# SonSang/dmesh_renderer

Hardware: AMD Instinct MI355X
Metric: fwd+bwd Mpixels/sec @1080p, 500k tris; grad max-abs-err vs ref (higher is better)
Workload: dtype f32

## Files before the change

dmesh_renderer_amd/csrc/dmr_api.hip:

```cpp
#include <algorithm>
#include <atomic>
#include <chrono>
#include <cstdio>
#include <cstdlib>
#include <cstring>
#include <functional>
#include <map>
#include <mutex>
#include <string>
#include <vector>

#include "dmr_kernels.hpp"

namespace {

thread_local std::string g_err;

int fail(const std::string& m) { g_err = m; return 1; }

#define DMR_HIP(expr)                                                                           \
    do {                                                                                        \
        hipError_t e_ = (expr);                                                                 \
        if (e_ != hipSuccess) return fail(std::string(#expr) + ": " + hipGetErrorString(e_));   \
    } while (0)

constexpr size_t ALIGN = 256;
inline size_t up(size_t n) { return (n + ALIGN - 1) & ~(ALIGN - 1); }

struct Carver {
    char* base; size_t off;
    explicit Carver(void* b) : base(reinterpret_cast<char*>(b)), off(0) {}
    template <class T> T* take(size_t count) {
        T* p = base ? reinterpret_cast<T*>(base + off) : nullptr;
        off += up(count * sizeof(T));
        return p;
    }
};

struct PointState { float4* vproj; };
struct FaceState { uint2* rect; float* key_depth; float* max_depth; uint32_t* tiles_touched; void* facerec; void* colrec; void* tetrec; };
struct ImageState {
    uint32_t* tile_count; uint32_t* tile_offset; uint32_t* tile_cursor; int* num_rendered;
    float* final_T; float* final_prev_T; uint32_t* n_contrib;
    uint32_t* tile_hits; uint32_t* tile_bound; uint32_t* scan_tmp; uint32_t* hit_offset; uint32_t* tile_used; unsigned long long* hit_total; uint32_t* tile_order;
    int32_t* first_face; int32_t* first_tet; int32_t* last_face; int32_t* last_tet; uint8_t* is_active;
    float* mats;
    int* seed;
    unsigned long long* mask_offset;
    dmr::TetSeq* seq;
};
struct BinningState {
    uint64_t* keys; uint32_t* face_list; uint32_t capacity; unsigned long long mask_offset, mask_first;
    char* base; unsigned long long seq_offset; uint32_t seq_steps;
};

size_t carve_point(void* b, size_t BP, PointState& s) { Carver c(b); s.vproj = c.take<float4>(BP); return c.off; }
size_t carve_face(void* b, size_t BF, size_t F, size_t T, bool tet, FaceState& s) {
    Carver c(b);
    s.rect = c.take<uint2>(BF); s.key_depth = c.take<float>(BF);
    s.max_depth = tet ? c.take<float>(BF) : nullptr;
    s.tiles_touched = c.take<uint32_t>(BF);
    s.facerec = s.colrec = s.tetrec = nullptr;
    if (tet) {
        s.facerec = c.take<char>(F * dmr::tet_facerec_bytes());
        s.colrec = c.take<char>(F * dmr::tet_colrec_bytes());
        s.tetrec = c.take<char>(T * dmr::tet_tetrec_bytes());
    }
    return c.off;
}
size_t carve_image(void* b, size_t B, size_t ntiles, size_t npix, bool tet, ImageState& s) {
    Carver c(b);
    s.mats = c.take<float>(64 * B);
    s.seed = c.take<int>(1);
    s.mask_offset = c.take<unsigned long long>(2);
    s.tile_count = c.take<uint32_t>(ntiles); s.tile_hits = c.take<uint32_t>(ntiles); s.tile_bound = c.take<uint32_t>(ntiles);
    s.scan_tmp = c.take<uint32_t>(dmr::scan_tmp_words((int)ntiles));
    s.hit_offset = c.take<uint32_t>(ntiles + 1); s.tile_used = c.take<uint32_t>(ntiles); s.hit_total = c.take<unsigned long long>(1);
    s.tile_offset = c.take<uint32_t>(ntiles + 1);
    s.tile_cursor = c.take<uint32_t>(ntiles); s.num_rendered = c.take<int>(1);
    s.tile_order = c.take<uint32_t>(ntiles);
    s.final_T = c.take<float>(npix); s.final_prev_T = c.take<float>(npix); s.n_contrib = c.take<uint32_t>(npix);
    if (tet) {
        s.first_face = c.take<int32_t>(npix); s.first_tet = c.take<int32_t>(npix);
        s.last_face = c.take<int32_t>(npix); s.last_tet = c.take<int32_t>(npix);
        s.is_active = c.take<uint8_t>(npix);
        s.seq = c.take<dmr::TetSeq>(1);
    } else {
        s.first_face = s.first_tet = s.last_face = s.last_tet = nullptr; s.is_active = nullptr;
        s.seq = nullptr;
    }
    return c.off;
}
size_t carve_binning(void* b, size_t R, size_t mask_tiles, size_t seq_tiles, size_t seq_steps, BinningState& s) {
    Carver c(b);
    s.face_list = c.take<uint32_t>(R); s.keys = c.take<uint64_t>(R);
    s.capacity = (uint32_t)std::min<size_t>(R, 0xffffffffu);
    s.mask_offset = c.off;
    s.mask_first = dmr::mask_first_slots(R, mask_tiles);
    if (mask_tiles && R > 0) c.take<uint4>(dmr::mask_slots(R, mask_tiles) * 256);
    s.base = reinterpret_cast<char*>(b); s.seq_offset = c.off; s.seq_steps = (uint32_t)seq_steps;
    if (seq_steps) c.take<char>(dmr::tet_seq_bytes(seq_tiles, seq_steps));
    return c.off;
}

struct Dims { int gx, gy, r0, r1, ntiles; size_t BP, BF, npix; };

dmr_scene canonical(const dmr_scene* s, const float* mats) {
    dmr_scene c = *s;
    const size_t n = 16 * (size_t)s->B;
    c.mv_mats = mats; c.proj_mats = mats + n; c.inv_mv_mats = mats + 2 * n; c.inv_proj_mats = mats + 3 * n;
    c.mats_transposed = 0;
    return c;
}

int check_scene(const dmr_scene* s, bool tet, Dims& d) {
    if (!s) return fail("null scene");
    if (s->B <= 0 || s->W <= 0 || s->H <= 0 || s->P < 0 || s->F < 0 || s->T < 0) return fail("bad dimensions");
    if ((int64_t)s->B * s->P > INT32_MAX || (int64_t)s->B * s->F > INT32_MAX || (int64_t)s->B * s->W * s->H > INT32_MAX)
        return fail("problem too large for 32-bit indexing");
    d.gx = (s->W + dmr::TILE - 1) / dmr::TILE;
    d.gy = (s->H + dmr::TILE - 1) / dmr::TILE;
    if (d.gx > 65535 || d.gy > 65535) return fail("image too large (tile coordinates must fit 16 bits)");
    d.r0 = s->row_begin; d.r1 = s->row_end;
    if (d.r0 == 0 && d.r1 == 0) d.r1 = d.gy;
    d.r0 = std::max(0, std::min(d.gy, d.r0));
    d.r1 = std::max(d.r0, std::min(d.gy, d.r1));
    d.ntiles = s->B * d.gx * d.gy;
    d.BP = (size_t)s->B * s->P; d.BF = (size_t)s->B * s->F; d.npix = (size_t)s->B * s->W * s->H;
    if (tet && s->F > 0 && s->P > 0 && (!s->tets || !s->face_tets || !s->tet_faces)) return fail("tet topology missing");
    if (tet && s->F >= (1 << 28)) return fail("too many faces for the tet renderer (face ids must fit 28 bits)");
    return 0;
}
// ... 38 lines not shown
    auto it = g_overflow.find(dev);
    if (it != g_overflow.end()) return it->second;
    if (!create) return nullptr;
    void* p = nullptr;
    if (hipHostMalloc(&p, 64, hipHostMallocCoherent | hipHostMallocPortable) != hipSuccess) return nullptr;
    *reinterpret_cast<volatile uint32_t*>(p) = 0u;
    return g_overflow[dev] = reinterpret_cast<uint32_t*>(p);
}

bool stream_is_capturing(hipStream_t st) {
    hipStreamCaptureStatus cs = hipStreamCaptureStatusNone;
    if (hipStreamIsCapturing(st, &cs) != hipSuccess) { (void)hipGetLastError(); return false; }
    return cs != hipStreamCaptureStatusNone;
}

struct SizeKey {
    int v[7];
    bool operator<(const SizeKey& o) const { return memcmp(v, o.v, sizeof(v)) < 0; }
};
struct SizeGuess { double rendered_per_face = 0.0, hits_per_face = 0.0; uint32_t* seq_steps = nullptr; };
std::mutex g_size_mu;
std::map<SizeKey, SizeGuess> g_size_cache;
std::atomic<uint64_t> g_redo_count{0};
int size_bucket(size_t BF) { int b = 0; while ((BF >> (b + 1)) != 0) b++; return b; }
SizeKey size_key(const dmr_scene* s, bool tet, const Dims& d) {
    return SizeKey{{s->B, s->W, s->H, d.r0, d.r1, tet ? 1 : 0, size_bucket(d.BF)}};
}
double lookup_estimate(const SizeKey& key, double SizeGuess::* field) {
    for (int db : {0, -1, 1}) {
        SizeKey k = key; k.v[6] += db;
        auto it = g_size_cache.find(k);
        if (it != g_size_cache.end() && it->second.*field > 0.0) return it->second.*field;
    }
    return 0.0;
}
uint64_t padded(uint64_t n) { return n + n / 4 + 4096; }

int run_forward(const dmr_scene* s, bool tet, const Dims& d, dmr_alloc_fn alloc, void* ctx, hipStream_t st,
                PointState& ps, FaceState& fs, ImageState& is, int* num_rendered,
                const std::function<void(const BinningState&)>& render) {
    PointState tp; FaceState tf; ImageState ti;
    void* pb = alloc(ctx, DMR_BUF_POINT, carve_point(nullptr, d.BP, tp));
    void* fb = alloc(ctx, DMR_BUF_FACE, carve_face(nullptr, d.BF, (size_t)s->F, (size_t)s->T, tet, tf));
    void* ib = alloc(ctx, DMR_BUF_IMAGE, carve_image(nullptr, (size_t)s->B, (size_t)d.ntiles, d.npix, tet, ti));
    if (!pb || !fb || !ib) return fail("scratch allocation failed");
    carve_point(pb, d.BP, ps);
    carve_face(fb, d.BF, (size_t)s->F, (size_t)s->T, tet, fs);
    carve_image(ib, (size_t)s->B, (size_t)d.ntiles, d.npix, tet, is);
    const bool async = (s->flags & DMR_FLAG_ASYNC) != 0 || stream_is_capturing(st);
    int dev = 0;
    DMR_HIP(hipGetDevice(&dev));
    uint32_t* overflow = overflow_word(dev, !async);

    auto front = [&](unsigned long long* host_R, uint32_t host_seq, uint64_t capacity, uint32_t* ovf) -> int {
        dmr::launch_project_verts(*s, ps.vproj, is.mats, is.tile_count, (size_t)(is.scan_tmp + dmr::SCAN_TMP_BUCKETS - is.tile_count), st);
        dmr::launch_setup_faces(*s, tet, ps.vproj, d.gx, d.gy, d.r0, d.r1, fs.rect, fs.key_depth, fs.max_depth,
                                fs.tiles_touched, is.tile_count, st);
        dmr::launch_scan_tiles(d.ntiles, is.tile_count, is.tile_offset, is.tile_cursor, is.num_rendered, host_R, host_seq, is.tile_order,
                               is.scan_tmp, (uint32_t)std::min<uint64_t>(capacity, 0xffffffffu), ovf, st);
        return 0;
    };
    size_t seq_steps = 0;
    if (tet) {
        std::lock_guard<std::mutex> lk(g_size_mu);
        SizeGuess& g = g_size_cache[size_key(s, tet, d)];
        if (!g.seq_steps && !async) {
            void* w = nullptr;
            if (hipHostMalloc(&w, 64, hipHostMallocCoherent | hipHostMallocPortable) == hipSuccess) {
                g.seq_steps = reinterpret_cast<uint32_t*>(w);
                *reinterpret_cast<volatile uint32_t*>(g.seq_steps) = 0u;
            } else (void)hipGetLastError();
        }
        if (g.seq_steps) {
            const uint64_t longest = *reinterpret_cast<volatile uint32_t*>(g.seq_steps);
            if (longest) {
                const uint64_t budget = 16ull << 30;
                const uint64_t per4 = dmr::tet_seq_bytes((size_t)d.ntiles, 4);
                seq_steps = (size_t)(std::min<uint64_t>((longest + longest / 4 + 4 + 3) / 4, std::max<uint64_t>(budget / std::max<uint64_t>(per4, 1), 1)) * 4);
            }
        }
    }
    auto rest = [&](uint64_t capacity) -> int {
        BinningState tb, bs;
        const size_t mask_tiles = tet ? 0 : (size_t)d.ntiles;
        void* bb = alloc(ctx, DMR_BUF_BINNING, carve_binning(nullptr, (size_t)capacity, mask_tiles, (size_t)d.ntiles, seq_steps, tb));
        if (!bb && (capacity > 0 || seq_steps > 0)) return fail("binning allocation failed");
        carve_binning(bb, (size_t)capacity, mask_tiles, (size_t)d.ntiles, seq_steps, bs);

        if (capacity > 0) {
            dmr::launch_scatter_faces(*s, d.gx, d.gy, fs.rect, fs.key_depth, fs.tiles_touched, is.tile_cursor, bs.keys,
                                      (uint32_t)capacity, tet ? nullptr : is.mask_offset, bs.mask_offset, bs.mask_first, st);
            if (d.ntiles > dmr::SCAN_SINGLE_MAX)
                dmr::launch_sort_tiles(d.ntiles, is.tile_offset, is.tile_order, bs.keys, bs.face_list, bs.capacity, st);
        }
        render(bs);
        return 0;
    };

    const SizeKey key = size_key(s, tet, d);
    uint64_t guess = 0;
    {
        std::lock_guard<std::mutex> lk(g_size_mu);
        const double per_face = lookup_estimate(key, &SizeGuess::rendered_per_face);
        if (per_face > 0.0) guess = std::min<uint64_t>(padded((uint64_t)(per_face * (double)d.BF)), 0x7fffffffu);
    }
    if (async) {
        if (!guess || !overflow)
            return fail("asynchronous / captured call without a size estimate: run one default (waiting) call with the same "
                        "view configuration first");
        if (front(nullptr, 0u, guess, overflow) || rest(guess)) return 1;
        *num_rendered = (int)guess;
        DMR_HIP(hipGetLastError());
        return 0;
    }
    SizeRead* sr = size_read();
    if (!sr) return fail("hipHostMalloc failed");
    const uint32_t seq = sr->next_seq();
    if (front(const_cast<unsigned long long*>(sr->word(0)), seq, ~0ull, nullptr)) return 1;
    if (guess && rest(guess)) return 1;
    unsigned long long R64 = 0;
    if (wait_size(sr->word(0), seq, st, &R64)) return 1;
    if (R64 > 0x7fffffffull) return fail("num_rendered overflows 31 bits");
    const int R = (int)R64;
    *num_rendered = R;
    if (!guess) {
        if (rest((uint64_t)R)) return 1;
    } else if ((uint64_t)R > guess) {
        g_redo_count.fetch_add(1, std::memory_order_relaxed);
        DMR_HIP(hipStreamSynchronize(st));
        if (front(nullptr, 0u, ~0ull, nullptr) || rest((uint64_t)R)) return 1;
    }
    {
        std::lock_guard<std::mutex> lk(g_size_mu);
        g_size_cache[key].rendered_per_face = (double)std::max(R, 1) / (double)std::max<size_t>(d.BF, 1);
    }
    DMR_HIP(hipGetLastError());
    return 0;
}

std::atomic<uint32_t> g_prof_mask{0};
struct ProfRec { int stage; hipEvent_t a, b; };
std::mutex g_prof_mu;
std::vector<ProfRec*> g_prof_live, g_prof_free;

}

namespace dmr {
StageScope::StageScope(int stage_, hipStream_t st_) : stage(stage_), st(st_), rec(nullptr) {
    if (!(g_prof_mask.load(std::memory_order_relaxed) & (1u << stage))) return;
    ProfRec* r = nullptr;
    {
        std::lock_guard<std::mutex> lk(g_prof_mu);
        if (!g_prof_free.empty()) { r = g_prof_free.back(); g_prof_free.pop_back(); }
    }
    if (!r) {
        r = new ProfRec();
        if (hipEventCreate(&r->a) != hipSuccess || hipEventCreate(&r->b) != hipSuccess) { delete r; return; }
    }
    r->stage = stage;
    (void)hipEventRecord(r->a, st);
    rec = r;
}
StageScope::~StageScope() {
    if (!rec) return;
    ProfRec* r = reinterpret_cast<ProfRec*>(rec);
    (void)hipEventRecord(r->b, st);
    std::lock_guard<std::mutex> lk(g_prof_mu);
    g_prof_live.push_back(r);
}
}

extern "C" {

void dmr_profile_enable(uint32_t mask) { g_prof_mask.store(mask); }

int dmr_profile_collect(double* ms, int64_t* launches) {
    std::vector<ProfRec*> live;
    {
        std::lock_guard<std::mutex> lk(g_prof_mu);
        live.swap(g_prof_live);
    }
    int rc = 0;
    for (ProfRec* r : live) {
// ... 253 lines not shown
}
__global__ void k_export_ranges(const uint32_t* off, const uint32_t* cnt, int64_t n, uint32_t* dst) {
    const int64_t i = (int64_t)blockIdx.x * blockDim.x + threadIdx.x;
    if (i >= n) return;
    const bool empty = cnt[i] == 0;
    dst[2 * i] = empty ? 0u : off[i];
    dst[2 * i + 1] = empty ? 0u : off[i + 1];
}
}

int64_t dmr_export(const dmr_scene* s, int is_tet, int num_rendered, const char* name, const void* point_buf,
                   const void* face_buf, const void* binning_buf, const void* image_buf, void* dst, int64_t cap,
                   void* stream) {
    Dims d;
    if (!name || check_scene(s, is_tet != 0, d)) return -1;
    hipStream_t st = reinterpret_cast<hipStream_t>(stream);
    PointState ps; FaceState fs; ImageState is; BinningState bs;
    carve_point(const_cast<void*>(point_buf), d.BP, ps);
    carve_face(const_cast<void*>(face_buf), d.BF, (size_t)s->F, (size_t)s->T, is_tet != 0, fs);
    carve_image(const_cast<void*>(image_buf), (size_t)s->B, (size_t)d.ntiles, d.npix, is_tet != 0, is);
    carve_binning(const_cast<void*>(binning_buf), (size_t)std::max(0, num_rendered), 0, 0, 0, bs);
    const std::string n(name);
    auto plain = [&](const void* src, size_t bytes) -> int64_t {
        if (dst && src && bytes) {
            if (hipMemcpyAsync(dst, src, std::min<size_t>(bytes, (size_t)cap), hipMemcpyDeviceToDevice, st) != hipSuccess) {
                g_err = "export copy failed";
                return -1;
            }
        }
        return (int64_t)bytes;
    };
    if (n == "image" || n == "ndc_z") {
        const size_t bytes = d.BP * (n == "image" ? 8 : 4);
        if (dst && d.BP && (size_t)cap >= bytes)
            k_export_vproj<<<dim3((unsigned)((d.BP + 255) / 256)), dim3(256), 0, st>>>(
                ps.vproj, (int64_t)d.BP, n == "image" ? 0 : 1, reinterpret_cast<float*>(dst));
        return (int64_t)bytes;
    }
    if (n == "ranges") {
        const size_t bytes = (size_t)d.ntiles * 8;
        if (dst && (size_t)cap >= bytes)
            k_export_ranges<<<dim3((unsigned)((d.ntiles + 255) / 256)), dim3(256), 0, st>>>(
                is.tile_offset, is.tile_count, d.ntiles, reinterpret_cast<uint32_t*>(dst));
        return (int64_t)bytes;
    }
    if (n == "key_depth") return plain(fs.key_depth, d.BF * 4);
    if (n == "max_depth") return is_tet ? plain(fs.max_depth, d.BF * 4) : -1;
    if (n == "tiles_touched") return plain(fs.tiles_touched, d.BF * 4);
    if (n == "face_list") return plain(bs.face_list, (size_t)std::max(0, num_rendered) * 4);
    if (n == "final_T") return plain(is.final_T, d.npix * 4);
    if (n == "final_prev_T") return plain(is.final_prev_T, d.npix * 4);
    if (n == "n_contrib") return plain(is.n_contrib, d.npix * 4);
    if (n == "tile_hits") return is_tet ? -1 : plain(is.tile_hits, (size_t)d.ntiles * 4);
    if (is_tet) {
        if (n == "first_face") return plain(is.first_face, d.npix * 4);
        if (n == "first_tet") return plain(is.first_tet, d.npix * 4);
        if (n == "last_face") return plain(is.last_face, d.npix * 4);
        if (n == "last_tet") return plain(is.last_tet, d.npix * 4);
        if (n == "is_active") return plain(is.is_active, d.npix);
        if (n == "tet_seq") return plain(is.seq, 8);
    }
    g_err = "unknown export item: " + n;
    return -1;
}

}
```

dmesh_renderer_amd/csrc/dmr_binning.hip:

```cpp
#include <algorithm>

#include "dmr_kernels.hpp"
#include "dmr_sort.hpp"

namespace dmr {

__device__ __forceinline__ float mat_at(const float* __restrict__ m, int k, bool transposed) {
    return m[transposed ? 4 * (k & 3) + (k >> 2) : k];
}

__global__ void __launch_bounds__(256)
k_project_verts(int B, int P, const float* __restrict__ verts, const float* __restrict__ mv_mats,
                const float* __restrict__ proj_mats, const float* __restrict__ inv_mv_mats,
                const float* __restrict__ inv_proj_mats, int transposed, const float* __restrict__ verts_depth,
                int W, int H, float4* __restrict__ vproj, float* __restrict__ mats,
                uint32_t* __restrict__ counters, uint32_t ncounters) {
    {
        const uint32_t per = (ncounters + gridDim.x - 1) / gridDim.x;
        const uint32_t z0 = min(ncounters, blockIdx.x * per), z1 = min(ncounters, z0 + per);
        for (uint32_t i = z0 + threadIdx.x; i < z1; i += 256) counters[i] = 0u;
    }
    if (blockIdx.x == 0) {
        for (int i = threadIdx.x; i < 64 * B; i += 256) {
            const int m = i / (16 * B), r = i % (16 * B);
// ... 100 lines not shown
        depth += a0.z;
        max_z = fmaxf(max_z, a1.z); min_z = fminf(min_z, a1.z); depth += a1.z;
        max_z = fmaxf(max_z, a2.z); min_z = fminf(min_z, a2.z); depth += a2.z;
        depth = depth / 3.0f;
        Rect r = {0, 0, 0, 0};
        if (!(max_z < -1.0f || min_z > 1.0f)) {
            r = tile_rect({a0.x, a0.y}, {a1.x, a1.y}, {a2.x, a2.y}, gx, gy, r0, r1);
            touched[it] = (r.maxy - r.miny) * (r.maxx - r.minx);
        }
        if (touched[it] == 0) r = {0, 0, 0, 0};
        auto map01 = [](float z) { float d = (z + 1.0f) * 0.5f; if (d < 0.0f) d = 0.0f; if (d > 1.0f) d = 1.0f; return d; };
        rr[it] = make_uint2(r.minx | (r.miny << 16), r.maxx | (r.maxy << 16));
        tiles_touched[idx] = touched[it];
        face_rect[idx] = rr[it];
        key_depth[idx] = touched[it] ? (TET ? map01(min_z) : map01(depth)) : 0.0f;
        if (TET) max_depth[idx] = touched[it] ? map01(max_z) : 0.0f;
    }
    const BinWindow w = bin_window<FPT>(s_box, view, rr, touched, mine, tid);
    const int nw = w.wx * w.wy;
    for (int t = tid; t < nw; t += 256) s_hist[t] = 0u;
    __syncthreads();
#pragma unroll
    for (int it = 0; it < FPT; it++) {
        if (touched[it] == 0) continue;
        const int64_t idx = base + it * 256 + tid;
        const uint32_t tb = (uint32_t)(idx / F) * gx * gy;
        const uint32_t minx = rr[it].x & 0xffffu, miny = rr[it].x >> 16, maxx = rr[it].y & 0xffffu, maxy = rr[it].y >> 16;
        if (touched[it] > BIG_RECT) {
            const uint32_t q = atomicAdd(&s_nbig, 1u);
            if (q < (uint32_t)BIG_MAX) { s_big[q] = BigFace{rr[it].x, rr[it].y, tb, 0u, 0u}; continue; }
        }
        if (w.lds && mine[it] && touched[it] <= BIG_RECT) {
            for (uint32_t y = miny; y < maxy; y++)
                for (uint32_t x = minx; x < maxx; x++) atomicAdd(&s_hist[(y - w.y0) * w.wx + (x - w.x0)], 1u);
        } else {
            for (uint32_t y = miny; y < maxy; y++)
                for (uint32_t x = minx; x < maxx; x++) atomicAdd(&tile_count[tb + y * gx + x], 1u);
        }
    }
    __syncthreads();
    for (int y = tid / 64; y < w.wy; y += 4)
        for (int x = tid % 64; x < w.wx; x += 64) {
            const uint32_t c = s_hist[y * w.wx + x];
            if (c) atomicAdd(&tile_count[(uint32_t)view * gx * gy + (uint32_t)(w.y0 + y) * gx + (uint32_t)(w.x0 + x)], c);
        }
    const uint32_t nbig = min(s_nbig, (uint32_t)BIG_MAX);
    for (uint32_t q = 0; q < nbig; q++) {
        const BigFace f = s_big[q];
        for (RectWalk t(f.rect_lo & 0xffffu, f.rect_lo >> 16, f.rect_hi & 0xffffu, f.rect_hi >> 16, (uint32_t)tid); t.valid(); t.next())
            atomicAdd(&tile_count[f.tile_base + t.y * gx + t.x], 1u);
    }
}

template <int FPT>
__global__ void __launch_bounds__(256)
k_scatter_faces_lds(int B, int F, int gx, int gy, const uint2* __restrict__ face_rect,
                    const float* __restrict__ key_depth, const uint32_t* __restrict__ tiles_touched,
                    uint32_t* __restrict__ tile_cursor, uint64_t* __restrict__ keys, uint32_t capacity,
                    unsigned long long* __restrict__ mask_offset_dst, unsigned long long mask_offset, unsigned long long mask_first) {
    if (mask_offset_dst && blockIdx.x == 0 && threadIdx.x == 0) { mask_offset_dst[0] = mask_offset; mask_offset_dst[1] = mask_first; }
    __shared__ uint32_t s_hist[LDS_HIST_MAX];
    __shared__ int s_box[4];
    __shared__ BigFace s_big[BIG_MAX];
    __shared__ uint32_t s_nbig;
    const int tid = threadIdx.x;
    if (tid == 0) s_nbig = 0u;
    const int64_t BF = (int64_t)B * F;
    const int64_t base = (int64_t)blockIdx.x * (256 * FPT);
    const int view = (int)(base / F);
    uint2 rr[FPT];
    uint32_t touched[FPT];
    bool mine[FPT];
#pragma unroll
    for (int it = 0; it < FPT; it++) {
        const int64_t idx = base + it * 256 + tid;
        touched[it] = idx < BF ? tiles_touched[idx] : 0u;
        rr[it] = touched[it] ? face_rect[idx] : make_uint2(0, 0);
        mine[it] = idx < BF && (int)(idx / F) == view;
    }
    const BinWindow w = bin_window<FPT>(s_box, view, rr, touched, mine, tid);
    const int nw = w.wx * w.wy;
    for (int t = tid; t < nw; t += 256) s_hist[t] = 0u;
    __syncthreads();
#pragma unroll
    for (int it = 0; it < FPT; it++) {
        if (!(w.lds && mine[it]) || touched[it] == 0 || touched[it] > BIG_RECT) continue;
        const uint32_t minx = rr[it].x & 0xffffu, miny = rr[it].x >> 16, maxx = rr[it].y & 0xffffu, maxy = rr[it].y >> 16;
        for (uint32_t y = miny; y < maxy; y++)
            for (uint32_t x = minx; x < maxx; x++) atomicAdd(&s_hist[(y - w.y0) * w.wx + (x - w.x0)], 1u);
    }
    __syncthreads();
    for (int y = tid / 64; y < w.wy; y += 4)
        for (int x = tid % 64; x < w.wx; x += 64) {
            const uint32_t c = s_hist[y * w.wx + x];
            if (c) s_hist[y * w.wx + x] = atomicAdd(&tile_cursor[(uint32_t)view * gx * gy + (uint32_t)(w.y0 + y) * gx + (uint32_t)(w.x0 + x)], c);
        }
    __syncthreads();
#pragma unroll
    for (int it = 0; it < FPT; it++) {
        if (touched[it] == 0) continue;
        const int64_t idx = base + it * 256 + tid;
        const int f = (int)(idx % F);
        const uint32_t tb = (uint32_t)(idx / F) * gx * gy;
        const uint32_t minx = rr[it].x & 0xffffu, miny = rr[it].x >> 16, maxx = rr[it].y & 0xffffu, maxy = rr[it].y >> 16;
        const uint64_t key = ((uint64_t)__float_as_uint(key_depth[idx]) << 32) | (uint32_t)f;
        if (touched[it] > BIG_RECT) {
            const uint32_t q = atomicAdd(&s_nbig, 1u);
            if (q < (uint32_t)BIG_MAX) { s_big[q] = BigFace{rr[it].x, rr[it].y, tb, (uint32_t)key, (uint32_t)(key >> 32)}; continue; }
        }
        const bool direct = !(w.lds && mine[it]) || touched[it] > BIG_RECT;
        for (uint32_t y = miny; y < maxy; y++)
            for (uint32_t x = minx; x < maxx; x++) {
                const uint32_t slot = direct ? atomicAdd(&tile_cursor[tb + y * gx + x], 1u)
                                             : atomicAdd(&s_hist[(y - w.y0) * w.wx + (x - w.x0)], 1u);
                if (slot < capacity) keys[slot] = key;
            }
    }
    __syncthreads();
    const uint32_t nbig = min(s_nbig, (uint32_t)BIG_MAX);
    for (uint32_t q = 0; q < nbig; q++) {
        const BigFace f = s_big[q];
        const uint64_t key = ((uint64_t)f.key_hi << 32) | f.key_lo;
        for (RectWalk t(f.rect_lo & 0xffffu, f.rect_lo >> 16, f.rect_hi & 0xffffu, f.rect_hi >> 16, (uint32_t)tid); t.valid();) {
            uint32_t tile[4], slot[4];
#pragma unroll
            for (int u = 0; u < 4; u++) {
                tile[u] = 0xffffffffu;
                if (t.valid()) { tile[u] = f.tile_base + t.y * gx + t.x; t.next(); }
            }
#pragma unroll
            for (int u = 0; u < 4; u++) slot[u] = tile[u] != 0xffffffffu ? atomicAdd(&tile_cursor[tile[u]], 1u) : 0xffffffffu;
#pragma unroll
            for (int u = 0; u < 4; u++) if (slot[u] < capacity) keys[slot[u]] = key;
        }
    }
}

constexpr int ORDER_BUCKETS = 64;
__device__ __forceinline__ int order_bucket(uint32_t n) { return ORDER_BUCKETS - 1 - (int)min(n >> 4, (uint32_t)(ORDER_BUCKETS - 1)); }
constexpr int ORDER_COPIES = 16;
constexpr int ORDER_CELLS = ORDER_BUCKETS * ORDER_COPIES;
__device__ __forceinline__ int order_cell(uint32_t n, int lane) { return order_bucket(n) * ORDER_COPIES + (lane & (ORDER_COPIES - 1)); }

constexpr int SCAN_BATCH = 8;

__device__ __forceinline__ uint32_t block_exclusive_scan(uint32_t local, int tid, uint32_t* wave_sum ) {
    const int lane = tid & 63, wave = tid >> 6;
    uint32_t incl = local;
#pragma unroll
    for (int d = 1; d < 64; d <<= 1) {
        uint32_t o = __shfl_up(incl, d, 64);
        if (lane >= d) incl += o;
    }
    if (lane == 63) wave_sum[wave] = incl;
    __syncthreads();
    if (tid < 64) {
        const uint32_t w = tid < 16 ? wave_sum[tid] : 0u;
        uint32_t wi = w;
#pragma unroll
        for (int d = 1; d < 16; d <<= 1) {
            uint32_t o = __shfl_up(wi, d, 64);
            if (tid >= d) wi += o;
        }
        if (tid < 16) wave_sum[tid] = wi - w;
        if (tid == 15) wave_sum[16] = wi;
    }
    __syncthreads();
    return wave_sum[wave] + incl - local;
}

constexpr int SCAN_SLAB = 1024 * SCAN_BATCH;

__device__ __forceinline__ void slab_load(uint32_t* __restrict__ slab, const uint32_t* __restrict__ src, int n, int tid) {
#pragma unroll
    for (int j = 0; j < SCAN_BATCH; j++) { const int i = j * 1024 + tid; slab[i] = i < n ? src[i] : 0u; }
}
__device__ __forceinline__ void slab_read(const uint32_t* __restrict__ slab, int tid, uint32_t (&c)[SCAN_BATCH]) {
    static_assert(SCAN_BATCH == 8, "two 16-byte LDS reads per thread");
    const uint4 lo = *reinterpret_cast<const uint4*>(slab + tid * SCAN_BATCH), hi = *reinterpret_cast<const uint4*>(slab + tid * SCAN_BATCH + 4);
    c[0] = lo.x; c[1] = lo.y; c[2] = lo.z; c[3] = lo.w; c[4] = hi.x; c[5] = hi.y; c[6] = hi.z; c[7] = hi.w;
}
__device__ __forceinline__ void slab_write_offsets(uint32_t* __restrict__ slab, int tid, uint32_t run, const uint32_t (&c)[SCAN_BATCH]) {
    uint32_t o[SCAN_BATCH];
#pragma unroll
    for (int j = 0; j < SCAN_BATCH; j++) { o[j] = run; run += c[j]; }
    *reinterpret_cast<uint4*>(slab + tid * SCAN_BATCH) = make_uint4(o[0], o[1], o[2], o[3]);
    *reinterpret_cast<uint4*>(slab + tid * SCAN_BATCH + 4) = make_uint4(o[4], o[5], o[6], o[7]);
}

__global__ void __launch_bounds__(1024)
k_scan_tiles(int n, const uint32_t* __restrict__ tile_count, uint32_t* __restrict__ tile_offset,
             uint32_t* __restrict__ tile_cursor, int* __restrict__ num_rendered, unsigned long long* __restrict__ host_num_rendered,
             uint32_t host_seq, uint32_t* __restrict__ tile_order, uint32_t capacity, uint32_t* __restrict__ overflow) {
    static_assert(ORDER_CELLS == 1024, "one counter cell per thread");
    __shared__ uint32_t wave_sum[17];
    __shared__ uint32_t bucket[ORDER_CELLS + 1];
    __shared__ __attribute__((aligned(16))) uint32_t slab[SCAN_SLAB];
    const int tid = threadIdx.x, lane = tid & 63;
    const int begin = tid * SCAN_BATCH;
    bucket[tid] = 0u;
    slab_load(slab, tile_count, n, tid);
    __syncthreads();
    uint32_t c[SCAN_BATCH], local = 0;
    slab_read(slab, tid, c);
#pragma unroll
    for (int j = 0; j < SCAN_BATCH; j++) {
        local += c[j];
        if (c[j]) atomicAdd(&bucket[order_cell(c[j], lane)], 1u);
    }
    const uint32_t run = block_exclusive_scan(local, tid, wave_sum);
    const uint32_t total = wave_sum[16];
    slab_write_offsets(slab, tid, run, c);
    __syncthreads();
    const uint32_t cell_base = block_exclusive_scan(bucket[tid], tid, wave_sum);
    bucket[tid] = cell_base;
    if (tid == 0) bucket[ORDER_CELLS] = wave_sum[16];
#pragma unroll
    for (int j = 0; j < SCAN_BATCH; j++) {
        const int i = j * 1024 + tid;
        if (i < n) { const uint32_t o = slab[i]; tile_offset[i] = o; tile_cursor[i] = o; }
    }
    __syncthreads();
// ... 216 lines not shown
void launch_setup_faces(const dmr_scene& s, bool tet, const float4* vproj, int gx, int gy, int r0, int r1,
                        uint2* face_rect, float* key_depth, float* max_depth, uint32_t* tiles_touched,
                        uint32_t* tile_count, hipStream_t st) {
    const int64_t n = (int64_t)s.B * s.F;
    if (n == 0) return;
    StageScope t(DMR_STAGE_SETUP_FACES, st);
    const int fpt = bin_fpt(n);
    dim3 grid((unsigned)((n + 256 * fpt - 1) / (256 * fpt))), block(256);
#define DMR_SETUP(TET, FPT) k_setup_faces_lds<TET, FPT><<<grid, block, 0, st>>>(s.B, s.P, s.F, s.faces, vproj, gx, gy, r0, r1, \
                                face_rect, key_depth, max_depth, tiles_touched, tile_count)
    if (tet) { if (fpt == 1) DMR_SETUP(true, 1); else if (fpt == 2) DMR_SETUP(true, 2); else DMR_SETUP(true, 4); }
    else { if (fpt == 1) DMR_SETUP(false, 1); else if (fpt == 2) DMR_SETUP(false, 2); else DMR_SETUP(false, 4); }
#undef DMR_SETUP
}

void launch_scan_tiles(int ntiles, const uint32_t* tile_count, uint32_t* tile_offset, uint32_t* tile_cursor,
                       int* num_rendered, unsigned long long* host_num_rendered, uint32_t host_seq, uint32_t* tile_order, uint32_t* scan_tmp,
                       uint32_t capacity, uint32_t* overflow, hipStream_t st) {
    StageScope t(DMR_STAGE_SCAN, st);
    if (ntiles <= SCAN_SINGLE_MAX) {
        k_scan_tiles<<<dim3(1), dim3(1024), 0, st>>>(ntiles, tile_count, tile_offset, tile_cursor, num_rendered, host_num_rendered, host_seq, tile_order,
                                                    capacity, overflow);
        return;
    }
    const int nblk = (ntiles + SCAN_BLOCK_TILES - 1) / SCAN_BLOCK_TILES;
    uint32_t* bucket = scan_tmp;
    uint32_t* blk_sum = scan_tmp + SCAN_TMP_BUCKETS;
    k_scan_tiles_partial<true><<<dim3(nblk), dim3(1024), 0, st>>>(ntiles, tile_count, nullptr, blk_sum, bucket);
    k_scan_tiles_blocks<<<dim3(1), dim3(1024), 0, st>>>(nblk, ntiles, blk_sum, bucket, tile_offset, num_rendered, host_num_rendered,
                                                        nullptr, nullptr, host_seq, capacity, overflow);
    k_scan_tiles_final<true><<<dim3(nblk), dim3(1024), 0, st>>>(ntiles, tile_count, nullptr, blk_sum, bucket, tile_offset, tile_cursor, tile_order);
}

size_t scan_tmp_words(int ntiles) { return SCAN_TMP_BUCKETS + (size_t)(ntiles + SCAN_BLOCK_TILES - 1) / SCAN_BLOCK_TILES + 1; }

void launch_scan_hits(int ntiles, const uint32_t* tile_hits, const uint32_t* tile_offset, uint32_t* hit_offset, uint32_t* tile_used,
                      unsigned long long* hit_total, unsigned long long* host_hit_total, uint32_t host_seq, uint32_t* scan_tmp, uint32_t capacity,
                      uint32_t* overflow, hipStream_t st) {
    StageScope t(DMR_STAGE_SCAN, st);
    if (ntiles <= SCAN_SINGLE_MAX) {
        k_scan_hits<<<dim3(1), dim3(1024), 0, st>>>(ntiles, tile_hits, tile_offset, hit_offset, tile_used, hit_total, host_hit_total, host_seq, capacity, overflow);
        return;
    }
    const int nblk = (ntiles + SCAN_BLOCK_TILES - 1) / SCAN_BLOCK_TILES;
    uint32_t* blk_sum = scan_tmp + SCAN_TMP_BUCKETS;
    k_scan_tiles_partial<false><<<dim3(nblk), dim3(1024), 0, st>>>(ntiles, tile_hits, tile_offset, blk_sum, nullptr);
    k_scan_tiles_blocks<<<dim3(1), dim3(1024), 0, st>>>(nblk, ntiles, blk_sum, nullptr, hit_offset, nullptr, nullptr, hit_total,
                                                        host_hit_total, host_seq, capacity, overflow);
    k_scan_tiles_final<false><<<dim3(nblk), dim3(1024), 0, st>>>(ntiles, tile_hits, tile_offset, blk_sum, nullptr, hit_offset, tile_used, nullptr);
}

void launch_scatter_faces(const dmr_scene& s, int gx, int gy, const uint2* face_rect, const float* key_depth,
                          const uint32_t* tiles_touched, uint32_t* tile_cursor, uint64_t* keys, uint32_t capacity,
                          unsigned long long* mask_offset_dst, unsigned long long mask_offset, unsigned long long mask_first, hipStream_t st) {
    const int64_t n = (int64_t)s.B * s.F;
    if (n == 0) return;
    StageScope t(DMR_STAGE_SCATTER, st);
    const int fpt = bin_fpt(n);
    const dim3 grid((unsigned)((n + 256 * fpt - 1) / (256 * fpt))), block(256);
#define DMR_SCATTER(FPT) k_scatter_faces_lds<FPT><<<grid, block, 0, st>>>(s.B, s.F, gx, gy, face_rect, key_depth, tiles_touched, \
                                                                         tile_cursor, keys, capacity, mask_offset_dst, mask_offset, mask_first)
    if (fpt == 1) DMR_SCATTER(1); else if (fpt == 2) DMR_SCATTER(2); else DMR_SCATTER(4);
#undef DMR_SCATTER
}

void launch_sort_tiles(int ntiles, const uint32_t* tile_offset, const uint32_t* tile_order, uint64_t* keys,
                       uint32_t* face_list, uint32_t capacity, hipStream_t st) {
    if (ntiles == 0) return;
    StageScope t(DMR_STAGE_SORT, st);
    k_sort_tiles<<<dim3((unsigned)std::min(ntiles, 256 * 64)), dim3(256), 0, st>>>((uint32_t)ntiles, tile_offset, tile_order, keys, face_list, capacity);
}

}
```

dmesh_renderer_amd/csrc/dmr_kernels.hpp:

```cpp
#pragma once

#include <hip/hip_runtime.h>
#include <stdint.h>

#include "../../include/dmesh_renderer_amd.h"
#include "dmr_device.hpp"

namespace dmr {

constexpr int VROW = 8;
constexpr int FROW = 2;
constexpr int HIT_GROUP = 4;
constexpr int HIT_BLOCK = 64 * HIT_GROUP;
__host__ __device__ inline uint32_t hit_slot_address(uint32_t rel) {
    return (rel & ~(uint32_t)(HIT_BLOCK - 1)) + (rel & (uint32_t)(HIT_GROUP - 1)) * 64u + ((rel & (uint32_t)(HIT_BLOCK - 1)) / (uint32_t)HIT_GROUP);
}

__host__ __device__ inline uint32_t record_bound(uint32_t h, uint32_t len) {
    if (h == 0u) return 0u;
    const uint32_t b = h + (uint32_t)(HIT_GROUP - 1) * (len < h ? len : h);
    return (b + (uint32_t)(HIT_BLOCK - 1)) & ~(uint32_t)(HIT_BLOCK - 1);
}
constexpr int SCAN_SINGLE_MAX = 8192;

struct StageScope {
    int stage; hipStream_t st; void* rec;
    StageScope(int stage, hipStream_t st);
    ~StageScope();
};

void launch_project_verts(const dmr_scene& s, float4* vproj, float* mats, uint32_t* counters, size_t ncounters,
                          hipStream_t st);
void launch_setup_faces(const dmr_scene& s, bool tet, const float4* vproj, int gx, int gy, int r0, int r1,
                        uint2* face_rect, float* key_depth, float* max_depth, uint32_t* tiles_touched,
                        uint32_t* tile_count, hipStream_t st);
constexpr int SCAN_TMP_BUCKETS = 128;
size_t scan_tmp_words(int ntiles);
__host__ __device__ inline unsigned long long host_size_word(uint32_t seq, unsigned long long size) {
    return ((unsigned long long)(seq & 0xffffffu) << 40) | (size < (1ull << 40) ? size : (1ull << 40) - 1ull);
}
void launch_scan_tiles(int ntiles, const uint32_t* tile_count, uint32_t* tile_offset, uint32_t* tile_cursor,
                       int* num_rendered, unsigned long long* host_num_rendered, uint32_t host_seq, uint32_t* tile_order, uint32_t* scan_tmp,
                       uint32_t capacity, uint32_t* overflow, hipStream_t st);
void launch_scatter_faces(const dmr_scene& s, int gx, int gy, const uint2* face_rect, const float* key_depth,
                          const uint32_t* tiles_touched, uint32_t* tile_cursor, uint64_t* keys, uint32_t capacity,
                          unsigned long long* mask_offset_dst, unsigned long long mask_offset, unsigned long long mask_first, hipStream_t st);
void launch_sort_tiles(int ntiles, const uint32_t* tile_offset, const uint32_t* tile_order, uint64_t* keys,
                       uint32_t* face_list, uint32_t capacity, hipStream_t st);

struct TriImageState {
    float* final_T; float* final_prev_T; uint32_t* n_contrib;
    uint32_t* tile_hits;
    uint32_t* tile_bound;
    const uint32_t* hit_offset;
    uint32_t* tile_used;
    const uint32_t* tile_order;
    const unsigned long long* mask_offset;
};
constexpr int MASK_CHUNK = 128;
inline size_t mask_first_slots(size_t list_capacity, size_t ntiles) { return list_capacity < ntiles ? list_capacity : ntiles; }
inline size_t mask_slots(size_t list_capacity, size_t ntiles) { return mask_first_slots(list_capacity, ntiles) + list_capacity / MASK_CHUNK + 1; }
struct alignas(16) HitRecord { uint32_t id; uint32_t pixel; float T; float dL_dalpha; };
void launch_tri_forward(const dmr_scene& s, int gx, int gy, int r0, int r1, const float4* vproj,
                        const uint32_t* tile_offset, uint64_t* keys, uint32_t* face_list, uint32_t capacity, TriImageState img,
                        float* out_color, float* out_depth, hipStream_t st);
void launch_scan_hits(int ntiles, const uint32_t* tile_hits, const uint32_t* tile_offset, uint32_t* hit_offset, uint32_t* tile_used,
                      unsigned long long* hit_total, unsigned long long* host_hit_total, uint32_t host_seq, uint32_t* scan_tmp, uint32_t capacity,
                      uint32_t* overflow, hipStream_t st);
struct HitRegions {
    uint32_t* hit_offset;
    unsigned long long* hit_total; unsigned long long* host_hit_total; uint32_t* overflow;
    uint32_t host_seq;
};
void launch_tri_backward_pix(const dmr_scene& s, int gx, int gy, int r0, int r1, const float4* vproj,
                             const uint32_t* tile_offset, const uint32_t* face_list, TriImageState img,
                             const float* dL_dcolor, const float* dL_ddepth, float4* pixrec, HitRecord* hits,
                             uint32_t capacity, float* work, size_t work_floats, HitRegions regions, hipStream_t st);
void launch_tri_backward_hits(const dmr_scene& s, int gx, int gy, const float4* vproj, const uint32_t* face_list, TriImageState img,
                              const float4* pixrec, const HitRecord* hits, uint32_t capacity, float* vrow, float* frow,
                              hipStream_t st);
void launch_tri_unpack(const dmr_scene& s, const float* vrow, const float* frow, float* dL_dverts,
                       float* dL_dvcolor, float* dL_dfopacity, float* dL_dvdepth, float* dL_dfintense,
                       hipStream_t st);

struct TetSeq {
    uint32_t max_steps;
    uint32_t cap_steps;
    unsigned long long offset;
};
inline size_t tet_seq_bytes(size_t ntiles, size_t cap_steps) { return ntiles * 4 * (cap_steps / 4) * 1024; }
struct TetImageState {
    float* final_log_T; float* final_prev_log_T; uint32_t* n_contrib;
    int32_t* first_face; int32_t* first_tet; int32_t* last_face; int32_t* last_tet; uint8_t* is_active;
    void* facerec; void* colrec; void* tetrec;
    int* seed;
    TetSeq* seq;
    char* binning;
};
size_t tet_facerec_bytes();
// ... 15 lines not shown
```

Before: 7238.

## Fuse tile prefix scan into the scatter kernel for small tile counts

When the tile count fits a single block, each scatter block now loads all per-tile counts, computes the exclusive scan and the tile ordering redundantly in its own registers and LDS, and adds the tile base offset to cursor-relative slots. This removes the separate scan_tiles launch and its dependency barrier between setup and scatter. In exchange every scatter block repeats the full scan, carries extra LDS and registers, and tile_cursor is moved so it is laid out just after the counts and is read as relative offsets.

```diff
diff --git a/dmesh_renderer_amd/csrc/dmr_api.hip b/dmesh_renderer_amd/csrc/dmr_api.hip
--- a/dmesh_renderer_amd/csrc/dmr_api.hip
+++ b/dmesh_renderer_amd/csrc/dmr_api.hip
@@ -74,10 +74,11 @@
     s.seed = c.take<int>(1);
     s.mask_offset = c.take<unsigned long long>(2);
     s.tile_count = c.take<uint32_t>(ntiles); s.tile_hits = c.take<uint32_t>(ntiles); s.tile_bound = c.take<uint32_t>(ntiles);
+    s.tile_cursor = c.take<uint32_t>(ntiles);
     s.scan_tmp = c.take<uint32_t>(dmr::scan_tmp_words((int)ntiles));
     s.hit_offset = c.take<uint32_t>(ntiles + 1); s.tile_used = c.take<uint32_t>(ntiles); s.hit_total = c.take<unsigned long long>(1);
     s.tile_offset = c.take<uint32_t>(ntiles + 1);
-    s.tile_cursor = c.take<uint32_t>(ntiles); s.num_rendered = c.take<int>(1);
+    s.num_rendered = c.take<int>(1);
     s.tile_order = c.take<uint32_t>(ntiles);
     s.final_T = c.take<float>(npix); s.final_prev_T = c.take<float>(npix); s.n_contrib = c.take<uint32_t>(npix);
     if (tet) {
@@ -222,12 +223,13 @@
     DMR_HIP(hipGetDevice(&dev));
     uint32_t* overflow = overflow_word(dev, !async);
 
-    auto front = [&](unsigned long long* host_R, uint32_t host_seq, uint64_t capacity, uint32_t* ovf) -> int {
+    auto front = [&](unsigned long long* host_R, uint32_t host_seq, uint64_t capacity, uint32_t* ovf, bool fused) -> int {
         dmr::launch_project_verts(*s, ps.vproj, is.mats, is.tile_count, (size_t)(is.scan_tmp + dmr::SCAN_TMP_BUCKETS - is.tile_count), st);
         dmr::launch_setup_faces(*s, tet, ps.vproj, d.gx, d.gy, d.r0, d.r1, fs.rect, fs.key_depth, fs.max_depth,
                                 fs.tiles_touched, is.tile_count, st);
-        dmr::launch_scan_tiles(d.ntiles, is.tile_count, is.tile_offset, is.tile_cursor, is.num_rendered, host_R, host_seq, is.tile_order,
-                               is.scan_tmp, (uint32_t)std::min<uint64_t>(capacity, 0xffffffffu), ovf, st);
+        if (!fused)
+            dmr::launch_scan_tiles(d.ntiles, is.tile_count, is.tile_offset, is.tile_cursor, is.num_rendered, host_R, host_seq, is.tile_order,
+                                   is.scan_tmp, (uint32_t)std::min<uint64_t>(capacity, 0xffffffffu), ovf, st);
         return 0;
     };
     size_t seq_steps = 0;
@@ -250,7 +252,7 @@
             }
         }
     }
-    auto rest = [&](uint64_t capacity) -> int {
+    auto rest = [&](uint64_t capacity, const dmr::FusedScan* fused) -> int {
         BinningState tb, bs;
         const size_t mask_tiles = tet ? 0 : (size_t)d.ntiles;
         void* bb = alloc(ctx, DMR_BUF_BINNING, carve_binning(nullptr, (size_t)capacity, mask_tiles, (size_t)d.ntiles, seq_steps, tb));
@@ -259,7 +261,7 @@
 
         if (capacity > 0) {
             dmr::launch_scatter_faces(*s, d.gx, d.gy, fs.rect, fs.key_depth, fs.tiles_touched, is.tile_cursor, bs.keys,
-                                      (uint32_t)capacity, tet ? nullptr : is.mask_offset, bs.mask_offset, bs.mask_first, st);
+                                      (uint32_t)capacity, tet ? nullptr : is.mask_offset, bs.mask_offset, bs.mask_first, fused, st);
             if (d.ntiles > dmr::SCAN_SINGLE_MAX)
                 dmr::launch_sort_tiles(d.ntiles, is.tile_offset, is.tile_order, bs.keys, bs.face_list, bs.capacity, st);
         }
@@ -274,11 +276,16 @@
         const double per_face = lookup_estimate(key, &SizeGuess::rendered_per_face);
         if (per_face > 0.0) guess = std::min<uint64_t>(padded((uint64_t)(per_face * (double)d.BF)), 0x7fffffffu);
     }
+    const bool fusable = d.ntiles <= dmr::SCAN_SINGLE_MAX && d.BF > 0;
+    auto fused_scan = [&](unsigned long long* host_R, uint32_t host_seq, uint32_t* ovf) {
+        return dmr::FusedScan{d.ntiles, is.tile_count, is.tile_offset, is.tile_order, is.num_rendered, host_R, host_seq, ovf};
+    };
     if (async) {
         if (!guess || !overflow)
             return fail("asynchronous / captured call without a size estimate: run one default (waiting) call with the same "
                         "view configuration first");
-        if (front(nullptr, 0u, guess, overflow) || rest(guess)) return 1;
+        const dmr::FusedScan fsc = fused_scan(nullptr, 0u, overflow);
+        if (front(nullptr, 0u, guess, overflow, fusable) || rest(guess, fusable ? &fsc : nullptr)) return 1;
         *num_rendered = (int)guess;
         DMR_HIP(hipGetLastError());
         return 0;
@@ -286,19 +293,21 @@
     SizeRead* sr = size_read();
     if (!sr) return fail("hipHostMalloc failed");
     const uint32_t seq = sr->next_seq();
-    if (front(const_cast<unsigned long long*>(sr->word(0)), seq, ~0ull, nullptr)) return 1;
-    if (guess && rest(guess)) return 1;
+    const bool fused = guess && fusable;
+    const dmr::FusedScan fsc = fused_scan(const_cast<unsigned long long*>(sr->word(0)), seq, nullptr);
+    if (front(const_cast<unsigned long long*>(sr->word(0)), seq, ~0ull, nullptr, fused)) return 1;
+    if (guess && rest(guess, fused ? &fsc : nullptr)) return 1;
     unsigned long long R64 = 0;
     if (wait_size(sr->word(0), seq, st, &R64)) return 1;
     if (R64 > 0x7fffffffull) return fail("num_rendered overflows 31 bits");
     const int R = (int)R64;
     *num_rendered = R;
     if (!guess) {
-        if (rest((uint64_t)R)) return 1;
+        if (rest((uint64_t)R, nullptr)) return 1;
     } else if ((uint64_t)R > guess) {
         g_redo_count.fetch_add(1, std::memory_order_relaxed);
         DMR_HIP(hipStreamSynchronize(st));
-        if (front(nullptr, 0u, ~0ull, nullptr) || rest((uint64_t)R)) return 1;
+        if (front(nullptr, 0u, ~0ull, nullptr, false) || rest((uint64_t)R, nullptr)) return 1;
     }
     {
         std::lock_guard<std::mutex> lk(g_size_mu);
@@ -658,6 +667,7 @@
     if (n == "final_prev_T") return plain(is.final_prev_T, d.npix * 4);
     if (n == "n_contrib") return plain(is.n_contrib, d.npix * 4);
     if (n == "tile_hits") return is_tet ? -1 : plain(is.tile_hits, (size_t)d.ntiles * 4);
+    if (n == "tile_order") return plain(is.tile_order, (size_t)d.ntiles * 4);
     if (is_tet) {
         if (n == "first_face") return plain(is.first_face, d.npix * 4);
         if (n == "first_tet") return plain(is.first_tet, d.npix * 4);
diff --git a/dmesh_renderer_amd/csrc/dmr_binning.hip b/dmesh_renderer_amd/csrc/dmr_binning.hip
--- a/dmesh_renderer_amd/csrc/dmr_binning.hip
+++ b/dmesh_renderer_amd/csrc/dmr_binning.hip
@@ -176,18 +176,160 @@
     }
 }
 
-template <int FPT>
+constexpr int ORDER_BUCKETS = 64;
+__device__ __forceinline__ int order_bucket(uint32_t n) { return ORDER_BUCKETS - 1 - (int)min(n >> 4, (uint32_t)(ORDER_BUCKETS - 1)); }
+__device__ __forceinline__ int order_bucket_or_empty(uint32_t n) { return n ? order_bucket(n) : ORDER_BUCKETS; }
+
+template <int NW = 16>
+__device__ __forceinline__ uint32_t block_exclusive_scan(uint32_t local, int tid, uint32_t* wave_sum ) {
+    const int lane = tid & 63, wave = tid >> 6;
+    uint32_t incl = local;
+#pragma unroll
+    for (int d = 1; d < 64; d <<= 1) {
+        uint32_t o = __shfl_up(incl, d, 64);
+        if (lane >= d) incl += o;
+    }
+    if (lane == 63) wave_sum[wave] = incl;
+    __syncthreads();
+    if (tid < 64) {
+        const uint32_t w = tid < NW ? wave_sum[tid] : 0u;
+        uint32_t wi = w;
+#pragma unroll
+        for (int d = 1; d < NW; d <<= 1) {
+            uint32_t o = __shfl_up(wi, d, 64);
+            if (tid >= d) wi += o;
+        }
+        if (tid < NW) wave_sum[tid] = wi - w;
+        if (tid == NW - 1) wave_sum[NW] = wi;
+    }
+    __syncthreads();
+    return wave_sum[wave] + incl - local;
+}
+
+
+__device__ __forceinline__ void fused_load(const uint32_t* __restrict__ tile_count, int n, int tid, uint4 (&c)[8]) {
+    static_assert(SCAN_SINGLE_MAX == 8 * 256 * 4, "eight 16-byte loads per thread cover every tile");
+    const uint4* __restrict__ q4 = reinterpret_cast<const uint4*>(tile_count);
+#pragma unroll
+    for (int j = 0; j < 8; j++) {
+        const int q = 256 * j + tid;
+        c[j] = 4 * q < n ? q4[q] : make_uint4(0u, 0u, 0u, 0u);
+    }
+#pragma unroll
+    for (int j = 0; j < 8; j++) {
+        const int i = 4 * (256 * j + tid);
+        if (i + 1 >= n) c[j].y = 0u;
+        if (i + 2 >= n) c[j].z = 0u;
+        if (i + 3 >= n) c[j].w = 0u;
+    }
+}
+
+__device__ __forceinline__ void fused_scan(const FusedScan& fs, const uint4 (&c)[8], uint32_t capacity, uint32_t* s_base,
+                                           uint32_t* s_wsum , uint32_t* s_scan , int tid) {
+    const int lane = tid & 63, wave = tid >> 6, n = fs.ntiles;
+    uint32_t qs[8], inc[8];
+#pragma unroll
+    for (int j = 0; j < 8; j++) { qs[j] = c[j].x + c[j].y + c[j].z + c[j].w; inc[j] = qs[j]; }
+#pragma unroll
+    for (int d = 1; d < 64; d <<= 1) {
+#pragma unroll
+        for (int j = 0; j < 8; j++) {
+            const uint32_t o = __shfl_up(inc[j], d, 64);
+            if (lane >= d) inc[j] += o;
+        }
+    }
+    if (lane == 63) {
+#pragma unroll
+        for (int j = 0; j < 8; j++) s_wsum[4 * j + wave] = inc[j];
+    }
+    __syncthreads();
+    uint32_t qb[8], run = 0;
+#pragma unroll
+    for (int j = 0; j < 8; j++) {
+        const uint4 w = *reinterpret_cast<const uint4*>(s_wsum + 4 * j);
+        qb[j] = run + (wave > 0 ? w.x : 0u) + (wave > 1 ? w.y : 0u) + (wave > 2 ? w.z : 0u) + inc[j] - qs[j];
+        run += w.x + w.y + w.z + w.w;
+    }
+    const uint32_t total = run;
+    if (!(tid & 1)) {
+#pragma unroll
+        for (int j = 0; j < 8; j++) s_base[(256 * j + tid) >> 1] = qb[j];
+    }
+    const int nq = (n + 3) / 4, per = (nq + (int)gridDim.x - 1) / (int)gridDim.x;
+    const int q0 = (int)blockIdx.x * per, q1 = min(nq, q0 + per);
+#pragma unroll
+    for (int j = 0; j < 8; j++) {
+        const int q = 256 * j + tid;
+        if (q < q0 || q >= q1) continue;
+        const uint4 o = make_uint4(qb[j], qb[j] + c[j].x, qb[j] + c[j].x + c[j].y, qb[j] + c[j].x + c[j].y + c[j].z);
+        if (4 * q + 3 < n) *reinterpret_cast<uint4*>(fs.tile_offset + 4 * q) = o;
+        else {
+            fs.tile_offset[4 * q] = o.x;
+            if (4 * q + 1 < n) fs.tile_offset[4 * q + 1] = o.y;
+            if (4 * q + 2 < n) fs.tile_offset[4 * q + 2] = o.z;
+        }
+    }
+    if (blockIdx.x == gridDim.x - 1 && tid == 0) {
+        fs.tile_offset[n] = total; *fs.num_rendered = (int)total;
+        if (fs.host_num_rendered) *fs.host_num_rendered = host_size_word(fs.host_seq, total);
+        if (fs.overflow && total > capacity) *fs.overflow = 1u;
+    }
+    for (int b = (int)blockIdx.x; b <= ORDER_BUCKETS; b += (int)gridDim.x) {
+        uint32_t v = 0;
+#pragma unroll
+        for (int j = 0; j < 8; j++) {
+            const int i = 4 * (256 * j + tid);
+            const uint32_t cc[4] = {c[j].x, c[j].y, c[j].z, c[j].w};
+#pragma unroll
+            for (int k = 0; k < 4; k++) {
+                const int bk = order_bucket_or_empty(cc[k]);
+                if (i + k < n) v += (bk < b ? 1u : 0u) + (bk == b ? 0x10000u : 0u);
+            }
+        }
+        const uint32_t ex = block_exclusive_scan<4>(v, tid, s_scan);
+        uint32_t pos = (s_scan[4] & 0xffffu) + (ex >> 16);
+        if (v >> 16) {
+#pragma unroll
+            for (int j = 0; j < 8; j++) {
+                const int i = 4 * (256 * j + tid);
+                const uint32_t cc[4] = {c[j].x, c[j].y, c[j].z, c[j].w};
+#pragma unroll
+                for (int k = 0; k < 4; k++)
+                    if (i + k < n && order_bucket_or_empty(cc[k]) == b) fs.tile_order[pos++] = (uint32_t)(i + k);
+            }
+        }
+        __syncthreads();
+    }
+    __syncthreads();
+}
+
+__device__ __forceinline__ uint32_t fused_offset(const uint32_t* s_base, const uint32_t* __restrict__ tile_count, uint32_t tile) {
+    const uint4* __restrict__ g = reinterpret_cast<const uint4*>(tile_count) + 2 * (tile >> 3);
+    const uint4 a = g[0], b = g[1];
+    const uint32_t r = tile & 7u;
+    return s_base[tile >> 3] + (r > 0 ? a.x : 0u) + (r > 1 ? a.y : 0u) + (r > 2 ? a.z : 0u) + (r > 3 ? a.w : 0u) +
+           (r > 4 ? b.x : 0u) + (r > 5 ? b.y : 0u) + (r > 6 ? b.z : 0u);
+}
+
+template <int FPT, bool FUSED>
 __global__ void __launch_bounds__(256)
 k_scatter_faces_lds(int B, int F, int gx, int gy, const uint2* __restrict__ face_rect,
                     const float* __restrict__ key_depth, const uint32_t* __restrict__ tiles_touched,
                     uint32_t* __restrict__ tile_cursor, uint64_t* __restrict__ keys, uint32_t capacity,
-                    unsigned long long* __restrict__ mask_offset_dst, unsigned long long mask_offset, unsigned long long mask_first) {
+                    unsigned long long* __restrict__ mask_offset_dst, unsigned long long mask_offset, unsigned long long mask_first,
+                    FusedScan fs) {
     if (mask_offset_dst && blockIdx.x == 0 && threadIdx.x == 0) { mask_offset_dst[0] = mask_offset; mask_offset_dst[1] = mask_first; }
     __shared__ uint32_t s_hist[LDS_HIST_MAX];
     __shared__ int s_box[4];
     __shared__ BigFace s_big[BIG_MAX];
     __shared__ uint32_t s_nbig;
+    __shared__ uint32_t s_base[FUSED ? SCAN_SINGLE_MAX / 8 : 1];
+    __shared__ __attribute__((aligned(16))) uint32_t s_wsum[FUSED ? 32 : 1];
+    __shared__ uint32_t s_scan[FUSED ? 5 : 1];
     const int tid = threadIdx.x;
+    uint4 cnt[8];
+    if (FUSED) fused_load(fs.tile_count, fs.ntiles, tid, cnt);
+    auto seg = [&](uint32_t tile) -> uint32_t { return FUSED ? fused_offset(s_base, fs.tile_count, tile) : 0u; };
     if (tid == 0) s_nbig = 0u;
     const int64_t BF = (int64_t)B * F;
     const int64_t base = (int64_t)blockIdx.x * (256 * FPT);
@@ -213,11 +355,13 @@
         for (uint32_t y = miny; y < maxy; y++)
             for (uint32_t x = minx; x < maxx; x++) atomicAdd(&s_hist[(y - w.y0) * w.wx + (x - w.x0)], 1u);
     }
+    if (FUSED) fused_scan(fs, cnt, capacity, s_base, s_wsum, s_scan, tid);
     __syncthreads();
     for (int y = tid / 64; y < w.wy; y += 4)
         for (int x = tid % 64; x < w.wx; x += 64) {
             const uint32_t c = s_hist[y * w.wx + x];
-            if (c) s_hist[y * w.wx + x] = atomicAdd(&tile_cursor[(uint32_t)view * gx * gy + (uint32_t)(w.y0 + y) * gx + (uint32_t)(w.x0 + x)], c);
+            const uint32_t tile = (uint32_t)view * gx * gy + (uint32_t)(w.y0 + y) * gx + (uint32_t)(w.x0 + x);
+            if (c) s_hist[y * w.wx + x] = seg(tile) + atomicAdd(&tile_cursor[tile], c);
         }
     __syncthreads();
 #pragma unroll
@@ -235,7 +379,7 @@
         const bool direct = !(w.lds && mine[it]) || touched[it] > BIG_RECT;
         for (uint32_t y = miny; y < maxy; y++)
             for (uint32_t x = minx; x < maxx; x++) {
-                const uint32_t slot = direct ? atomicAdd(&tile_cursor[tb + y * gx + x], 1u)
+                const uint32_t slot = direct ? seg(tb + y * gx + x) + atomicAdd(&tile_cursor[tb + y * gx + x], 1u)
                                              : atomicAdd(&s_hist[(y - w.y0) * w.wx + (x - w.x0)], 1u);
                 if (slot < capacity) keys[slot] = key;
             }
@@ -253,45 +397,18 @@
                 if (t.valid()) { tile[u] = f.tile_base + t.y * gx + t.x; t.next(); }
             }
 #pragma unroll
-            for (int u = 0; u < 4; u++) slot[u] = tile[u] != 0xffffffffu ? atomicAdd(&tile_cursor[tile[u]], 1u) : 0xffffffffu;
+            for (int u = 0; u < 4; u++) slot[u] = tile[u] != 0xffffffffu ? seg(tile[u]) + atomicAdd(&tile_cursor[tile[u]], 1u) : 0xffffffffu;
 #pragma unroll
             for (int u = 0; u < 4; u++) if (slot[u] < capacity) keys[slot[u]] = key;
         }
     }
 }
 
-constexpr int ORDER_BUCKETS = 64;
-__device__ __forceinline__ int order_bucket(uint32_t n) { return ORDER_BUCKETS - 1 - (int)min(n >> 4, (uint32_t)(ORDER_BUCKETS - 1)); }
 constexpr int ORDER_COPIES = 16;
 constexpr int ORDER_CELLS = ORDER_BUCKETS * ORDER_COPIES;
 __device__ __forceinline__ int order_cell(uint32_t n, int lane) { return order_bucket(n) * ORDER_COPIES + (lane & (ORDER_COPIES - 1)); }
 
 constexpr int SCAN_BATCH = 8;
-
-__device__ __forceinline__ uint32_t block_exclusive_scan(uint32_t local, int tid, uint32_t* wave_sum ) {
-    const int lane = tid & 63, wave = tid >> 6;
-    uint32_t incl = local;
-#pragma unroll
-    for (int d = 1; d < 64; d <<= 1) {
-        uint32_t o = __shfl_up(incl, d, 64);
-        if (lane >= d) incl += o;
-    }
-    if (lane == 63) wave_sum[wave] = incl;
-    __syncthreads();
-    if (tid < 64) {
-        const uint32_t w = tid < 16 ? wave_sum[tid] : 0u;
-        uint32_t wi = w;
-#pragma unroll
-        for (int d = 1; d < 16; d <<= 1) {
-            uint32_t o = __shfl_up(wi, d, 64);
-            if (tid >= d) wi += o;
-        }
-        if (tid < 16) wave_sum[tid] = wi - w;
-        if (tid == 15) wave_sum[16] = wi;
-    }
-    __syncthreads();
-    return wave_sum[wave] + incl - local;
-}
 
 constexpr int SCAN_SLAB = 1024 * SCAN_BATCH;
 
@@ -614,15 +731,18 @@
 
 void launch_scatter_faces(const dmr_scene& s, int gx, int gy, const uint2* face_rect, const float* key_depth,
                           const uint32_t* tiles_touched, uint32_t* tile_cursor, uint64_t* keys, uint32_t capacity,
-                          unsigned long long* mask_offset_dst, unsigned long long mask_offset, unsigned long long mask_first, hipStream_t st) {
+                          unsigned long long* mask_offset_dst, unsigned long long mask_offset, unsigned long long mask_first,
+                          const FusedScan* fused, hipStream_t st) {
     const int64_t n = (int64_t)s.B * s.F;
     if (n == 0) return;
     StageScope t(DMR_STAGE_SCATTER, st);
     const int fpt = bin_fpt(n);
     const dim3 grid((unsigned)((n + 256 * fpt - 1) / (256 * fpt))), block(256);
-#define DMR_SCATTER(FPT) k_scatter_faces_lds<FPT><<<grid, block, 0, st>>>(s.B, s.F, gx, gy, face_rect, key_depth, tiles_touched, \
-                                                                         tile_cursor, keys, capacity, mask_offset_dst, mask_offset, mask_first)
-    if (fpt == 1) DMR_SCATTER(1); else if (fpt == 2) DMR_SCATTER(2); else DMR_SCATTER(4);
+    const FusedScan fs = fused ? *fused : FusedScan{};
+#define DMR_SCATTER(FPT, FUSED) k_scatter_faces_lds<FPT, FUSED><<<grid, block, 0, st>>>(s.B, s.F, gx, gy, face_rect, key_depth, \
+                                    tiles_touched, tile_cursor, keys, capacity, mask_offset_dst, mask_offset, mask_first, fs)
+    if (fused) { if (fpt == 1) DMR_SCATTER(1, true); else if (fpt == 2) DMR_SCATTER(2, true); else DMR_SCATTER(4, true); }
+    else { if (fpt == 1) DMR_SCATTER(1, false); else if (fpt == 2) DMR_SCATTER(2, false); else DMR_SCATTER(4, false); }
 #undef DMR_SCATTER
 }
 
diff --git a/dmesh_renderer_amd/csrc/dmr_kernels.hpp b/dmesh_renderer_amd/csrc/dmr_kernels.hpp
--- a/dmesh_renderer_amd/csrc/dmr_kernels.hpp
+++ b/dmesh_renderer_amd/csrc/dmr_kernels.hpp
@@ -42,9 +42,14 @@
 void launch_scan_tiles(int ntiles, const uint32_t* tile_count, uint32_t* tile_offset, uint32_t* tile_cursor,
                        int* num_rendered, unsigned long long* host_num_rendered, uint32_t host_seq, uint32_t* tile_order, uint32_t* scan_tmp,
                        uint32_t capacity, uint32_t* overflow, hipStream_t st);
+struct FusedScan {
+    int ntiles; const uint32_t* tile_count; uint32_t* tile_offset; uint32_t* tile_order;
+    int* num_rendered; unsigned long long* host_num_rendered; uint32_t host_seq; uint32_t* overflow;
+};
 void launch_scatter_faces(const dmr_scene& s, int gx, int gy, const uint2* face_rect, const float* key_depth,
                           const uint32_t* tiles_touched, uint32_t* tile_cursor, uint64_t* keys, uint32_t capacity,
-                          unsigned long long* mask_offset_dst, unsigned long long mask_offset, unsigned long long mask_first, hipStream_t st);
+                          unsigned long long* mask_offset_dst, unsigned long long mask_offset, unsigned long long mask_first,
+                          const FusedScan* fused, hipStream_t st);
 void launch_sort_tiles(int ntiles, const uint32_t* tile_offset, const uint32_t* tile_order, uint64_t* keys,
                        uint32_t* face_list, uint32_t capacity, hipStream_t st);
 
```

Result: faster. 7359 (median of 6 runs) (+1.7%).
